# Jaureguy760/HaploHyped-VarAwareML

Measured on AMD Instinct MI355X. Metric: variants/sec encode+compress, 3M-variant x 2.5k-sample VCF, higher is better.
Workload: dtype u8

## Files before the change

### haplohyped_varawareml_amd/csrc/api.hip

```cpp
#include "common.h"
#include <chrono>
#include <vector>
#include <stdarg.h>
#include <stdio.h>
#include <string.h>
#include <stdlib.h>

static thread_local char g_err[512] = "";

void hhgt_set_error(const char *fmt, ...)
{
    va_list ap;
    va_start(ap, fmt);
    vsnprintf(g_err, sizeof(g_err), fmt, ap);
    va_end(ap);
}

extern "C" const char *hhgt_last_error(void) { return g_err; }
extern "C" const char *hhgt_version(void) { return "hhgt 0.1 (gfx950)"; }

extern "C" int hhgt_device_count(void)
{
    int n = 0;
    if (hipGetDeviceCount(&n) != hipSuccess) return 0;
// ... 68 lines not shown
    }
    if (rc == HHGT_OK) rc = c->counters.ensure(sizeof(DevCounters));
    if (rc != HHGT_OK) {
        hhgt_ctx_destroy(c);
        return rc;
    }
    *out = c;
    return HHGT_OK;
}

extern "C" void hhgt_ctx_destroy(hhgt_ctx *c)
{
    if (!c) return;
    hipSetDevice(c->device);
    hipDeviceSynchronize();
    DevBuf *bufs[] = {&c->slots, &c->counts, &c->prefix, &c->nl, &c->scan_tmp, &c->l_soff, &c->l_lend, &c->l_pos,
                      &c->l_refalt, &c->l_flags, &c->l_keep, &c->l_kidx, &c->l_cnew, &c->l_crun, &c->k_soff,
                      &c->k_lend, &c->k_meta, &c->redo_list, &c->redo_flag, &c->run_first, &c->run_names,
                      &c->counters, &c->cursor, &c->result, &c->dec_bad, &c->oh_ovl, &c->oh_lut, &c->crc_x2n,
                      &c->ld_bits};
    for (DevBuf *b : bufs) b->release();
    for (auto &w : c->cw) {
        DevBuf *wb[] = {&w.lz_scratch, &w.lz_csize, &w.lz_flags, &w.fr_bsize, &w.fr_csize, &w.fr_flags};
        for (DevBuf *b : wb) b->release();
        if (w.lz_done) hipEventDestroy(w.lz_done);
        if (w.fr_done) hipEventDestroy(w.fr_done);
    }
    if (c->h_counters) hipHostFree(c->h_counters);
    if (c->h_result_pinned) hipHostFree(c->h_result_pinned);
    for (auto &p : c->pending) {
        hipEventDestroy(p.a);
// ... 217 lines not shown
        return HHGT_ERR_ARG;
    }
    if (L->S > 0 && !d_G) {
        hhgt_set_error("encode: d_G is NULL");
        return HHGT_ERR_ARG;
    }
    const int rc = parse_region_host(region, rf);
    rf->keep_multi = c->keep_multi;
    return rc;
}

static int encode_stage_index(hhgt_ctx *c, const uint8_t *text, uint64_t nbytes, uint32_t n_regions, uint32_t min_line, uint32_t S,
                              DevCounters *cnt, hipStream_t st)
{
    TRY(c->slots.ensure((size_t)n_regions * INDEX_CAP * 4));
    TRY(c->counts.ensure((size_t)n_regions * 4));
    TRY(c->prefix.ensure(((size_t)n_regions + 1) * 4));
    TRY(c->scan_tmp.ensure(2 * scan_tmp_elems(n_regions) * 4));
    TRY(launch_index_newlines(text, nbytes, c->slots.as<uint32_t>(), c->counts.as<uint32_t>(), n_regions, min_line, S, c->index_mode, cnt, st));
    TRY(launch_scan_exclusive_u32_pair(c->counts.as<uint32_t>(), c->prefix.as<uint32_t>(), nullptr, nullptr, n_regions,
                                       c->scan_tmp.as<uint32_t>(), c->scan_tmp.cap / 4, st));
    return HHGT_OK;
}

static int encode_stage_rest(hhgt_ctx *c, const uint8_t *text, uint64_t nbytes, uint32_t n_regions, uint32_t max_lines,
                             const RegionFilter &rf, const LayoutDev &L, const uint64_t *d_cursor, void *d_G, void *d_P, uint32_t *d_start, uint32_t *d_stop,
                             uint8_t *d_ref, uint8_t *d_alt, DevCounters *cnt, hipStream_t st)
{
    const uint32_t *d_nlines = c->prefix.as<uint32_t>() + n_regions;
    const size_t nl4 = ((size_t)max_lines + 1) * 4;
    TRY(c->nl.ensure(nl4));
    TRY(c->scan_tmp.ensure(2 * scan_tmp_elems(max_lines) * 4));
    DevBuf *per_line[] = {&c->l_soff, &c->l_lend, &c->l_pos, &c->l_refalt, &c->l_flags, &c->l_keep,
                          &c->l_kidx, &c->l_cnew, &c->l_crun, &c->k_soff, &c->k_lend, &c->k_meta,
                          &c->redo_list, &c->redo_flag};
    for (DevBuf *b : per_line) TRY(b->ensure(nl4));
    TRY(c->run_first.ensure(MAX_CHROM_RUNS * 8));
    TRY(c->run_names.ensure(MAX_CHROM_RUNS * 32));
    {
        StageTimer t(c, st, HHGT_STAGE_INDEX);
        TRY(launch_compact_newlines(c->slots.as<uint32_t>(), c->counts.as<uint32_t>(), c->prefix.as<uint32_t>(),
                                    n_regions, c->nl.as<uint32_t>(), max_lines, st));
        t.stop();
    }
    if (max_lines == 0) return HHGT_OK;
    {
        StageTimer t(c, st, HHGT_STAGE_FIXED);
        TRY(launch_parse_fixed(text, nbytes, c->nl.as<uint32_t>(), d_nlines, max_lines, rf, L.S,
                               c->l_soff.as<uint32_t>(), c->l_lend.as<uint32_t>(), c->l_pos.as<uint32_t>(),
                               c->l_refalt.as<uint32_t>(), c->l_flags.as<uint32_t>(), c->l_keep.as<uint32_t>(),
                               c->l_cnew.as<uint32_t>(), c->index_mode, cnt, st));
        TRY(launch_scan_exclusive_u32_pair(c->l_keep.as<uint32_t>(), c->l_kidx.as<uint32_t>(), c->l_cnew.as<uint32_t>(),
                                           c->l_crun.as<uint32_t>(), max_lines, c->scan_tmp.as<uint32_t>(), c->scan_tmp.cap / 4, st));
        TRY(launch_compact_kept(text, nbytes, c->nl.as<uint32_t>(), d_nlines, max_lines, c->l_soff.as<uint32_t>(),
                                c->l_lend.as<uint32_t>(), c->l_pos.as<uint32_t>(), c->l_refalt.as<uint32_t>(),
                                c->l_flags.as<uint32_t>(), c->l_kidx.as<uint32_t>(), c->l_crun.as<uint32_t>(),
                                c->k_soff.as<uint32_t>(), c->k_lend.as<uint32_t>(), c->k_meta.as<uint32_t>(),
                                c->redo_list.as<uint32_t>(), c->redo_flag.as<uint32_t>(), c->run_first.as<uint64_t>(), c->run_names.as<uint8_t>(),
                                MAX_CHROM_RUNS, d_cursor, L.v_capacity, L.ring, d_start, d_stop, d_ref, d_alt, cnt, d_P != nullptr, st));
        t.stop();
    }
    if (L.S > 0) {
        StageTimer t(c, st, HHGT_STAGE_ENCODE);
// ... 463 lines not shown
    TRY(planes_columns(lay, col0, n_cols, &L, &pg));
    const uint64_t chunk_nbytes = (uint64_t)L.Sc * L.Vc * 2ull, col_bytes = chunk_nbytes * L.n_sc;
    const uint8_t *g = d_G ? static_cast<const uint8_t *>(d_G) + (uint64_t)col0 * col_bytes : nullptr;
    return compress_impl(c, g, d_P, pg, (uint64_t)n_cols * L.n_sc, chunk_nbytes, 2, 8192, format, d_dst, dst_cap, d_chunk_off, total_bytes,
                         stream);
}

extern "C" int hhgt_reserve(hhgt_ctx *c, uint64_t text_bytes, uint32_t max_lines, uint64_t n_chunks, uint64_t chunk_nbytes, int typesize,
                            int blocksize)
{
    if (!c) return HHGT_ERR_ARG;
    HIP_TRY(hipSetDevice(c->device));
    if (text_bytes) {
        const uint32_t n_regions = (uint32_t)((text_bytes + 1 + INDEX_REGION - 1) / INDEX_REGION);
        TRY(c->slots.ensure((size_t)n_regions * INDEX_CAP * 4));
        TRY(c->counts.ensure((size_t)n_regions * 4));
        TRY(c->prefix.ensure(((size_t)n_regions + 1) * 4));
        const size_t st_el = scan_tmp_elems(n_regions) > scan_tmp_elems(max_lines) ? scan_tmp_elems(n_regions) : scan_tmp_elems(max_lines);
        TRY(c->scan_tmp.ensure(2 * st_el * 4));
        const size_t nl4 = ((size_t)max_lines + 1) * 4;
        TRY(c->nl.ensure(nl4));
        DevBuf *per_line[] = {&c->l_soff, &c->l_lend, &c->l_pos, &c->l_refalt, &c->l_flags, &c->l_keep, &c->l_kidx, &c->l_cnew, &c->l_crun,
                              &c->k_soff, &c->k_lend, &c->k_meta, &c->redo_list, &c->redo_flag};
        for (DevBuf *b : per_line) TRY(b->ensure(nl4));
        TRY(c->run_first.ensure(MAX_CHROM_RUNS * 8));
        TRY(c->run_names.ensure(MAX_CHROM_RUNS * 32));
        TRY(c->result.ensure(sizeof(hhgt_encode_result)));
    }
    if (n_chunks) {
        TRY(check_codec_args(chunk_nbytes, typesize, blocksize, HHGT_BLOSC2));
        blocksize = effective_blocksize(chunk_nbytes, typesize, blocksize);
        uint32_t nblocks, nwaves;
        size_t slot;
        codec_geometry(chunk_nbytes, typesize, blocksize, &nblocks, &nwaves, &slot);
        const uint64_t n_streams = n_chunks * nblocks * nwaves;
        hhgt_ctx::CodecWs &w = c->cw[0];
        TRY(w.lz_scratch.ensure((size_t)n_streams * slot));
// ... 71 lines not shown
        HIP_TRY(hipStreamDestroy(reinterpret_cast<hipStream_t>(stream)));
    }
    return HHGT_OK;
}

extern "C" int hhgt_set_index_mode(hhgt_ctx *c, int mode)
{
    if (!c || mode < -1 || mode > 2) {
        hhgt_set_error("index mode must be -1 (default), 0 (scan), 1 (hop) or 2 (walk)");
        return HHGT_ERR_ARG;
    }
    c->index_mode = mode;
    return HHGT_OK;
}

extern "C" int hhgt_set_keep_multiallelic(hhgt_ctx *c, int on)
{
    if (!c) return HHGT_ERR_ARG;
    c->keep_multi = on ? 1 : 0;
    return HHGT_OK;
}

__global__ void k_count_nonzero_u32(const uint32_t *__restrict__ v, uint64_t n, unsigned long long *out)
{
    uint64_t i = (uint64_t)blockIdx.x * blockDim.x + threadIdx.x;
    const unsigned long long m = __ballot(i < n && v[i] != 0u);
    if ((threadIdx.x & 63u) == 0u && m) atomicAdd(out, (unsigned long long)__builtin_popcountll(m));
}

extern "C" int hhgt_inflate_members(hhgt_ctx *c, const void *d_src, uint64_t src_bytes, const uint64_t *d_comp_off,
// ... 263 lines not shown
```

### haplohyped_varawareml_amd/csrc/common.h

```cpp
#pragma once
#include <hip/hip_runtime.h>
#include <stdint.h>
#include <stddef.h>
#include <string>
#include <vector>
#include "../../include/hhgt.h"

#define HHGT_WAVE 64
#ifdef HHGT_ENC_PRIO
#define HHGT_WAVE_PRIO() __builtin_amdgcn_s_setprio(HHGT_ENC_PRIO)
#else
#define HHGT_WAVE_PRIO()
#endif

#ifdef __HIPCC__
__device__ __forceinline__ uint32_t wave_scan_sum_dpp(uint32_t x, uint32_t lane)
{
    x += (uint32_t)__builtin_amdgcn_update_dpp(0, (int)x, 0x111, 0xf, 0xf, false);
    x += (uint32_t)__builtin_amdgcn_update_dpp(0, (int)x, 0x112, 0xf, 0xf, false);
    x += (uint32_t)__builtin_amdgcn_update_dpp(0, (int)x, 0x114, 0xf, 0xf, false);
    x += (uint32_t)__builtin_amdgcn_update_dpp(0, (int)x, 0x118, 0xf, 0xf, false);
    const uint32_t t0 = (uint32_t)__builtin_amdgcn_readlane((int)x, 15);
    const uint32_t t1 = (uint32_t)__builtin_amdgcn_readlane((int)x, 31) + t0;
    const uint32_t t2 = (uint32_t)__builtin_amdgcn_readlane((int)x, 47) + t1;
// ... 97 lines not shown
    *bi = rem - (rem / g.bpr) * g.bpr;
}

struct DevBuf {
    void *p = nullptr;
    size_t cap = 0;
    int ensure(size_t bytes);
    void release();
    template <typename T> T *as() const { return reinterpret_cast<T *>(p); }
};

struct hhgt_ctx {
    int device = 0;
    hipDeviceProp_t prop;
    DevBuf slots, counts, prefix, nl, scan_tmp;
    DevBuf l_soff, l_lend, l_pos, l_refalt, l_flags, l_keep, l_kidx, l_cnew, l_crun;
    DevBuf k_soff, k_lend, k_meta, redo_list, redo_flag, run_first, run_names;
    DevBuf counters;
    DevBuf cursor;
    DevBuf result;
    struct CodecWs {
        DevBuf lz_scratch, lz_csize, lz_flags, fr_bsize, fr_csize, fr_flags;
        uint32_t lz_tag = 0;
        hipEvent_t lz_done = nullptr, fr_done = nullptr;
        bool fr_pending = false;
    } cw[2];
    uint64_t cmp_seq = 0;
    hipStream_t frame_stream = nullptr;
    DevBuf dec_bad, oh_ovl, oh_lut, crc_x2n;
    DevBuf ld_bits;
// ... 19 lines not shown
    hhgt_ctx *ctx;
    hipStream_t st;
    int stage;
    hipEvent_t a = nullptr, b = nullptr;
    StageTimer(hhgt_ctx *c, hipStream_t s, int stage_);
    void stop();
};
int hhgt_profile_collect(hhgt_ctx *ctx);

int launch_scan_exclusive_u32(const uint32_t *d_in, uint32_t *d_out, uint64_t n, uint32_t *d_tmp,
                              size_t tmp_elems, hipStream_t st);
int launch_scan_exclusive_u32_pair(const uint32_t *in_a, uint32_t *out_a, const uint32_t *in_b, uint32_t *out_b, uint64_t n,
                                   uint32_t *d_tmp, size_t tmp_elems, hipStream_t st);
size_t scan_tmp_elems(uint64_t n);

int launch_index_newlines(const uint8_t *d_text, uint64_t n, uint32_t *d_slots, uint32_t *d_counts,
                          uint32_t n_regions, uint32_t min_line, uint32_t S, int mode, DevCounters *d_cnt, hipStream_t st);
int index_mode_default();
int launch_compact_newlines(const uint32_t *d_slots, const uint32_t *d_counts, const uint32_t *d_prefix,
                            uint32_t n_regions, uint32_t *d_nl, uint32_t max_lines, hipStream_t st);
int launch_parse_fixed(const uint8_t *d_text, uint64_t n, const uint32_t *d_nl, const uint32_t *d_nlines,
                       uint32_t max_lines, const RegionFilter &region, uint32_t S, uint32_t *l_soff, uint32_t *l_lend,
                       uint32_t *l_pos, uint32_t *l_refalt, uint32_t *l_flags, uint32_t *l_keep,
                       uint32_t *l_cnew, int mode, DevCounters *d_cnt, hipStream_t st);
int launch_compact_kept(const uint8_t *d_text, uint64_t n, const uint32_t *d_nl, const uint32_t *d_nlines, uint32_t max_lines,
                        const uint32_t *l_soff, const uint32_t *l_lend,
                        const uint32_t *l_pos, const uint32_t *l_refalt, const uint32_t *l_flags,
                        const uint32_t *l_kidx, const uint32_t *l_crun, uint32_t *k_soff, uint32_t *k_lend,
                        uint32_t *k_meta, uint32_t *redo_list, uint32_t *redo_flag, uint64_t *run_first, uint8_t *run_names,
                        uint32_t max_runs, const uint64_t *d_cursor, uint64_t v_capacity, uint32_t ring, uint32_t *d_start,
                        uint32_t *d_stop, uint8_t *d_ref, uint8_t *d_alt, DevCounters *d_cnt, bool strided, hipStream_t st);

int launch_encode_tiles(const uint8_t *d_text, uint64_t n, const uint32_t *k_soff, const uint32_t *k_meta,
                        uint32_t n_lines_bound, const uint64_t *d_cursor, LayoutDev lay, int8_t *d_G,
                        uint32_t *redo_list, uint32_t *redo_flag, DevCounters *d_cnt, hipStream_t st);
int launch_encode_general(const uint8_t *d_text, uint64_t n, const uint32_t *k_soff, const uint32_t *k_lend,
// ... 57 lines not shown
```

### haplohyped_varawareml_amd/csrc/index.hip

```cpp
#include "common.h"

typedef uint32_t u32x4_unaligned __attribute__((ext_vector_type(4), aligned(1)));
typedef uint32_t u32x4_t __attribute__((ext_vector_type(4)));

__device__ __forceinline__ uint32_t nl_mask4(uint32_t x)
{
    uint32_t t = x ^ 0x0A0A0A0Au;
    uint32_t z = ~(((t & 0x7F7F7F7Fu) + 0x7F7F7F7Fu) | t | 0x7F7F7F7Fu);
    return (((z >> 7) * 0x01020408u) >> 24) & 0xFu;
}

__global__ __launch_bounds__(256) void k_index_newlines(const uint8_t *__restrict__ text, uint64_t n,
                                                        uint32_t *__restrict__ slots,
                                                        uint32_t *__restrict__ counts, uint32_t n_regions,
                                                        DevCounters *cnt)
{
    HHGT_WAVE_PRIO();
    const uint32_t lane = threadIdx.x & 63u;
    const uint32_t r = blockIdx.x * 4u + (threadIdx.x >> 6);
    if (r >= n_regions) return;
    const bool virt = n > 0 && text[n - 1] != '\n';
    const uint64_t rbase = (uint64_t)r * INDEX_REGION;
    uint32_t *my = slots + (size_t)r * INDEX_CAP;
    uint32_t wcount = 0;
// ... 61 lines not shown
    const uint32_t q = (off >> 2) & 3u;
    const uint32_t d = q == 0u ? v.x : (q == 1u ? v.y : (q == 2u ? v.z : v.w));
    return ((uint32_t)__builtin_amdgcn_readlane((int)d, (int)(off >> 4)) >> (8u * (off & 3u))) & 0xFFu;
}

__device__ __forceinline__ uint32_t head_kth(uint32_t m16, uint32_t cum, uint32_t k)
{
    const unsigned long long b = __builtin_amdgcn_ballot_w64(cum < k && cum + (uint32_t)__popc(m16) >= k);
    const int l = __builtin_ctzll(b);
    uint32_t m = (uint32_t)__builtin_amdgcn_readlane((int)m16, l);
    const uint32_t r = k - (uint32_t)__builtin_amdgcn_readlane((int)cum, l);
    for (uint32_t i = 1; i < r; ++i) m &= m - 1u;
    return 16u * (uint32_t)l + (uint32_t)__builtin_ctz(m);
}

#ifndef WALK_BATCH
#define WALK_BATCH 1
#endif
#ifndef WALK_PF
#define WALK_PF 0
#endif
template <int U, bool WALK>
__global__ __launch_bounds__(256) void k_index_hop(const uint8_t *__restrict__ text, uint64_t n, uint32_t *__restrict__ slots,
                                                   uint32_t *__restrict__ counts, uint32_t n_regions, uint32_t skip, uint32_t S,
                                                   DevCounters *cnt, uint32_t HOP_K)
{
    HHGT_WAVE_PRIO();
    const uint32_t lane = threadIdx.x & 63u;
    const uint32_t w = (uint32_t)__builtin_amdgcn_readfirstlane((int)(blockIdx.x * 4u + (threadIdx.x >> 6)));
    const uint32_t r_first = w * HOP_K;
    if (r_first >= n_regions) return;
    const uint32_t r_cnt = n_regions - r_first < HOP_K ? n_regions - r_first : HOP_K;
    const bool virt = n > 0 && text[n - 1] != '\n';
    const uint64_t beg = (uint64_t)r_first * INDEX_REGION;
    uint64_t endw = beg + (uint64_t)r_cnt * INDEX_REGION;
    if (endw > n + 1) endw = n + 1;
    const uint64_t last_term = virt ? n : n - 1;
    uint32_t cntv = 0;
    bool overflow = false;
    uint64_t pos = beg;
    uint64_t cand = 0, fb = 0;
    bool have_cand = false;
    uint64_t est_len = 0, pf_wb = 0;
    bool pf_valid = false;
    u32x4_t pf = u32x4_t{0u, 0u, 0u, 0u};
    auto record = [&](uint64_t q) {
        const uint32_t rr = (uint32_t)(q / INDEX_REGION), local = rr - r_first;
        const uint32_t c = (uint32_t)__builtin_amdgcn_readlane((int)cntv, (int)local);
        if (c < INDEX_CAP) {
            if (lane == 0) slots[(size_t)rr * INDEX_CAP + c] = (uint32_t)q;
        } else
            overflow = true;
        cntv += lane == local ? 1u : 0u;
    };
    bool no_batch = false, bat_off = false;
    uint32_t bat_fail = 0;
    uint64_t head_p = 0;
    bool cand_batch = false;
    bool rehead = false;
    while (have_cand || pos < endw) {
        if (WALK && WALK_BATCH && have_cand && !no_batch && !bat_off && est_len != 0ull && cand >= 40ull && cand + 3ull * est_len + 216ull <= n) {
            const uint32_t g = lane >> 4, li = lane & 15u;
            const uint64_t L0 = est_len;
            const uint8_t *wbase = text + (cand - 40ull);
            const uint64_t voff = (uint64_t)g * L0 + 16ull * li;
// ... 26 lines not shown
#pragma unroll
            for (uint32_t i = 0; i < 8u; ++i) m9 = i < r1 ? (m9 & (m9 - 1u)) : m9;
            const uint32_t j9 = (uint32_t)__builtin_ctz(m9 | 0x10000u) & 15u;
            const uint32_t pw = (uint32_t)__builtin_amdgcn_update_dpp(0, (int)v.w, 0x111, 0xf, 0xf, false);
            const uint32_t ptb = (uint32_t)__builtin_amdgcn_update_dpp(0, (int)tbm, 0x111, 0xf, 0xf, false);
            const uint32_t tb20 = (tbm << 4) | (ptb >> 12);
            const bool tab8 = ((tb20 >> (j9 + 1u)) & 1u) != 0u;
            const uint32_t ix = j9 + 2u, di = ix >> 2;
            const uint32_t w0 = di == 0u ? pw : (di == 1u ? v.x : (di == 2u ? v.y : (di == 3u ? v.z : v.w)));
            const uint32_t w1 = di == 0u ? v.x : (di == 1u ? v.y : (di == 2u ? v.z : v.w));
            const uint32_t gt2 = __builtin_amdgcn_alignbyte(w1, w0, ix & 3u) & 0xFFFFu;
            const bool ok9 = has9 && tab8 && gt2 == 0x5447u;
            const uint32_t t9 = l0 + j9;
            const unsigned long long b9 = __builtin_amdgcn_ballot_w64(ok9);
            uint64_t expected = cand, fbx = fb, exp_head = head_p;
            bool exp_batch = cand_batch;
            bool stop = false, handed = false;
            uint32_t advanced = 0;
#pragma unroll
            for (int k = 0; k < 4; ++k) {
                if (stop || handed) continue;
                const uint64_t nlpos = cand - 40ull + (uint64_t)k * L0 + og[k];
                const bool cr = vg[k] && og[k] != 0u && head_byte(v, 256u * (uint32_t)k + og[k] - 1u) == '\r';
                if (!vg[k] || nlpos != expected || cr) {
                    handed = true;
                    continue;
                }
                exp_head = expected;
                exp_batch = true;
                if (expected >= endw) {
                    stop = true;
                    continue;
                }
                const uint32_t bits = (uint32_t)(b9 >> (16 * k)) & 0xFFFFu;
                if (bits == 0u || ((nl2 >> (16 * k)) & 0xFFFFull) != 0ull) {
                    have_cand = false;
                    pos = expected;
                    handed = true;
                    expected = ~0ull;
                    continue;
                }
                record(expected);
                ++advanced;
                const int l9 = 16 * k + __builtin_ctz(bits);
                const uint32_t t9s = (uint32_t)__builtin_amdgcn_readlane((int)t9, l9);
                const uint64_t soff = cand - 40ull + (uint64_t)k * L0 + t9s + 1ull;
                const uint64_t nxt = soff + 4ull * S - 1ull;
                est_len = nxt - expected;
                expected = nxt;
                fbx = soff + 2ull * S - 17ull;
            }
            if (stop) break;
            if (expected != ~0ull) {
                if (expected > last_term) {
                    have_cand = false;
                    pos = fbx;
                    if (pos > last_term) pos = last_term;
                } else {
                    cand = expected;
                    fb = fbx > last_term ? last_term : fbx;
                    have_cand = true;
                }
                head_p = exp_head;
                cand_batch = exp_batch;
            }
            no_batch = handed;
            bat_fail = advanced ? 0u : bat_fail + 1u;
            bat_off = bat_fail >= 2u;
            continue;
        }
        no_batch = false;
        bool found = false, nb_have = false, have_head = false;
        uint32_t nb_reg = 0, ho = 15u;
        uint64_t p = 0;
        u32x4_t hd = u32x4_t{0u, 0u, 0u, 0u};
        if (WALK && have_cand) {
            have_cand = false;
            uint32_t c15 = 0, c14 = 0;
            const bool use_pf = pf_valid && cand >= pf_wb + 15ull && cand <= pf_wb + 79ull;
            pf_valid = false;
            if (use_pf || cand + 1009ull <= n) {
                if (use_pf) {
                    hd = pf;
                    ho = (uint32_t)(cand - pf_wb);
                } else
                    hd = *reinterpret_cast<const u32x4_unaligned *>(text + (cand - 15ull) + 16ull * lane);
                const uint64_t pred = cand + est_len;
                if (WALK_PF && est_len != 0ull && pred + 977ull <= n && cand < endw) {
// ... 2 lines not shown
                    pf_valid = true;
                }
                c15 = head_byte(hd, ho);
                c14 = head_byte(hd, ho - 1u);
                have_head = true;
            } else if (cand < n) {
                c15 = text[cand];
                c14 = text[cand - 1];
            } else if (cand == n && virt) {
                c15 = 0x0Au;
                c14 = text[n - 1];
            }
            if (c15 == 0x0Au && c14 != '\r') {
                found = true;
                p = cand;
            } else if (cand_batch) {
                cand_batch = false;
                rehead = true;
                found = true;
                have_head = false;
                p = head_p;
            } else {
                pos = fb;
                continue;
            }
        } else {
        const uint64_t a0 = pos & ~15ull;
        uint32_t any[U];
        u32x4_t v[U];
#pragma unroll
// ... 43 lines not shown
                    if (j < 15u && g0 + 16 <= n) {
                        const uint32_t k = j + 1u, dw = k >> 2;
                        const uint32_t xd = dw == 0u ? x0 : (dw == 1u ? x1 : (dw == 2u ? x2 : x3));
                        nb_reg = (xd >> (8u * (k & 3u))) & 0xFFu;
                        nb_have = true;
                    }
                }
            }
        }
        if (!found) {
            pos = a0 + (uint64_t)U * 1024u;
            continue;
        }
        }
        if (!rehead) {
            if (p >= endw) break;
            record(p);
        } else
            no_batch = true;
        rehead = false;
        bool hopped = false;
        if (WALK) {
            if (!have_head && p >= 15ull && p + 1009ull <= n) {
                hd = *reinterpret_cast<const u32x4_unaligned *>(text + (p - 15ull) + 16ull * lane);
                have_head = true;
            }
            if (have_head) {
                const uint64_t wb = p - (uint64_t)ho;
                const uint32_t nb = head_byte(hd, ho + 1u);
                const uint32_t l0 = 16u * lane;
                const uint32_t keep = l0 > ho ? 0xFFFFu : (l0 + 15u <= ho ? 0u : (0xFFFFu << (ho - l0 + 1u)) & 0xFFFFu);
                if (nb == '#' || nb == 0x0Au) {
// ... 6 lines not shown
                        const int l = __builtin_ctzll(nlb);
                        pos = wb + 16ull * (uint64_t)l + (uint64_t)__builtin_ctz((uint32_t)__builtin_amdgcn_readlane((int)nlm, l));
                        hopped = true;
                    } else {
                        const uint32_t tbm = eq_mask16(hd, 0x09090909u) & keep;
                        const uint32_t tc = (uint32_t)__popc(tbm);
                        const uint32_t incl = wave_scan_sum_dpp(tc, lane);
                        const uint32_t total = (uint32_t)__builtin_amdgcn_readlane((int)incl, 63);
                        if (total >= 9u) {
                            const uint32_t t8 = head_kth(tbm, incl - tc, 8u), t9 = head_kth(tbm, incl - tc, 9u);
                            const uint64_t soff = wb + t9 + 1ull;
                            const uint64_t lo = soff + 2ull * S - 17ull;
                            const bool gt = t9 - t8 == 3u && head_byte(hd, t8 + 1u) == 'G' && head_byte(hd, t8 + 2u) == 'T';
                            if (gt && soff + 4ull * S - 1ull <= last_term) {
                                cand = soff + 4ull * S - 1ull;
                                fb = lo;
                                have_cand = true;
                                est_len = cand - p;
                                head_p = p;
                                cand_batch = false;
                            } else {
                                pos = lo;
                            }
                            hopped = true;
                        }
                    }
                }
            }
        }
        if (!hopped) {
            uint32_t nb = 0x0Au;
            if (nb_have) nb = nb_reg;
            else if (p + 1 < n) nb = text[p + 1];
            pos = p + 1 + ((nb == '#' || nb == 0x0Au || nb == '\r') ? 0u : skip);
        }
        if (pos > last_term) pos = p + 1 > last_term ? p + 1 : last_term;
        if (have_cand && fb > last_term) fb = p + 1 > last_term ? p + 1 : last_term;
    }
    if (overflow && lane == 0) atomicAdd(&cnt->err_density, 1ull);
    if (lane < r_cnt) counts[r_first + lane] = cntv < INDEX_CAP ? cntv : INDEX_CAP;
}

__global__ __launch_bounds__(256) void k_compact_newlines(const uint32_t *__restrict__ slots,
                                                          const uint32_t *__restrict__ counts,
                                                          const uint32_t *__restrict__ prefix,
                                                          uint32_t n_regions, uint32_t *__restrict__ nl,
                                                          uint32_t max_lines)
{
    HHGT_WAVE_PRIO();
    uint32_t r = blockIdx.x * blockDim.x + threadIdx.x;
    if (r >= n_regions) return;
    uint32_t c = counts[r], p = prefix[r];
    const uint32_t *my = slots + (size_t)r * INDEX_CAP;
    for (uint32_t k = 0; k < c && p + k < max_lines; ++k) nl[p + k] = my[k];
}

__global__ __launch_bounds__(256) void k_parse_fixed(const uint8_t *__restrict__ text, uint64_t n,
                                                     const uint32_t *__restrict__ nl, const uint32_t *__restrict__ d_nlines,
                                                     uint32_t max_lines, const RegionFilter rfv, uint32_t S,
                                                     uint32_t *__restrict__ l_soff, uint32_t *__restrict__ l_lend,
                                                     uint32_t *__restrict__ l_pos, uint32_t *__restrict__ l_refalt,
                                                     uint32_t *__restrict__ l_flags, uint32_t *__restrict__ l_keep,
                                                     uint32_t *__restrict__ l_cnew, DevCounters *cnt, uint32_t hop_skip)
{
    HHGT_WAVE_PRIO();
    __shared__ uint32_t stage[256][17];
    const RegionFilter *rf = &rfv;
    const uint32_t i = blockIdx.x * blockDim.x + threadIdx.x;
    const uint32_t n_found = *d_nlines;
    const uint32_t n_lines = n_found < max_lines ? n_found : max_lines;
    if (i == 0) {
        cnt->n_lines = n_found;
        cnt->err_lines = n_found > max_lines ? (unsigned long long)(n_found - max_lines) : 0ull;
    }
    if (blockIdx.x * blockDim.x >= n_lines) {
        if (i < max_lines) l_keep[i] = l_cnew[i] = 0u;
        return;
    }
    uint32_t flags = 0;
    uint32_t s = 0, e = 0;
    bool staged = false;
    if (i < n_lines) {
        s = i ? nl[i - 1] + 1u : 0u;
        e = nl[i];
        staged = (uint64_t)s + 64ull <= n;
        if (staged) {
            u32x4_unaligned c[4];
#pragma unroll
            for (int k = 0; k < 4; ++k) c[k] = *reinterpret_cast<const u32x4_unaligned *>(text + s + 16 * k);
#pragma unroll
            for (int k = 0; k < 4; ++k) {
                stage[threadIdx.x][4 * k + 0] = c[k].x;
                stage[threadIdx.x][4 * k + 1] = c[k].y;
                stage[threadIdx.x][4 * k + 2] = c[k].z;
                stage[threadIdx.x][4 * k + 3] = c[k].w;
            }
        }
    }
    __syncthreads();
    const uint8_t *mine = reinterpret_cast<const uint8_t *>(stage[threadIdx.x]);
    auto rd = [&](uint32_t x) -> uint32_t { return (staged && x - s < 64u) ? (uint32_t)mine[x - s] : (uint32_t)text[x]; };
    uint32_t soff = 0, pos0 = 0, refalt = 0, gtidx = 0, stride = 0;
    if (i < n_lines) {
        if (e > s && rd(e - 1u) == '\r') --e;
        soff = e;
        if (e > s && rd(s) != '#') {
            flags = LF_RECORD;
            uint32_t fs[10];
            uint32_t nf = 0;
            uint32_t p = s;
            fs[0] = s;
            while (p < e && nf < 9) {
                if (rd(p) == '\t') fs[++nf] = p + 1;
                ++p;
            }
            bool bad = false;
            uint32_t fe[9];
#pragma unroll
            for (int k = 0; k < 9; ++k) fe[k] = (uint32_t)k < nf ? fs[k + 1] - 1u : e;
            if (nf < 7 || (S > 0 && nf < 9)) bad = true;
            if (!bad) {
                unsigned long long pos = 0;
                if (fe[1] == fs[1]) bad = true;
                for (uint32_t q = fs[1]; q < fe[1]; ++q) {
                    uint32_t c = rd(q);
                    if (c < '0' || c > '9') {
                        bad = true;
                        break;
                    }
// ... 17 lines not shown
                        bool snp = reflen == 1 && altlen == 1 && (a == 'A' || a == 'C' || a == 'G' || a == 'T');
                        if (rf->keep_multi && reflen == 1 && altlen > 1 && (altlen & 1u)) {
                            snp = true;
                            for (uint32_t q = 0; snp && q < altlen; ++q) {
                                const uint32_t ch = rd(fs[4] + q);
                                snp = (q & 1u) ? ch == ',' : (ch == 'A' || ch == 'C' || ch == 'G' || ch == 'T');
                            }
                        }
                        if (!snp)
                            flags |= LF_DROP_FILTER;
                        else {
                            pos0 = (uint32_t)(pos - 1ull);
                            refalt = rd(fs[3]) | (a << 8);
                            if (S > 0) {
                                uint32_t q = fs[8], k = 0;
                                bool found = false;
                                while (q <= fe[8]) {
                                    uint32_t q2 = q;
                                    while (q2 < fe[8] && rd(q2) != ':') ++q2;
                                    if (q2 - q == 2 && rd(q) == 'G' && rd(q + 1u) == 'T') {
                                        found = true;
                                        break;
                                    }
                                    ++k;
                                    q = q2 + 1;
                                }
                                if (!found || k > 0xFFFu) bad = true;
                                gtidx = k;
                                soff = fs[9];
                                if (!bad) {
                                    flags |= LF_KEEP;
                                    if (k == 0 && fe[8] - fs[8] == 2 && e - soff == 4u * S - 1u) flags |= LF_FAST;
// ... 2 lines not shown
                                        if (wd >= 5u && wd <= 8u) stride = wd;
                                    }
                                }
                            } else {
                                flags |= LF_KEEP;
                            }
                        }
                    }
                }
            }
            if (bad) flags = LF_RECORD | LF_MALFORMED;
            bool cnew = true;
            if (i > 0) {
                uint32_t ps = i > 1 ? nl[i - 2] + 1u : 0u;
                uint32_t pe = nl[i - 1];
                const bool pstaged = threadIdx.x > 0u && (uint64_t)ps + 64ull <= n;
                const uint8_t *prev = reinterpret_cast<const uint8_t *>(stage[threadIdx.x > 0u ? threadIdx.x - 1u : 0u]);
                auto rdp = [&](uint32_t x) -> uint32_t { return (pstaged && x - ps < 64u) ? (uint32_t)prev[x - ps] : (uint32_t)text[x]; };
                if (pe > ps && rdp(ps) != '#') {
                    uint32_t q = 0;
                    cnew = false;
                    for (;;) {
                        uint32_t a = fs[0] + q < e ? rd(fs[0] + q) : '\t';
                        uint32_t b = ps + q < pe ? rdp(ps + q) : '\t';
                        if (a != b) {
                            cnew = true;
                            break;
                        }
                        if (a == '\t') break;
                        ++q;
                    }
                }
            }
// ... 131 lines not shown
{
    static const int m = [] {
        if (const char *e = getenv("HHGT_INDEX_MODE")) return atoi(e);
        if (const char *e = getenv("HHGT_INDEX_HOP")) return atoi(e) ? 2 : 0;
        return 2;
    }();
    return m < 0 ? 0 : (m > 2 ? 2 : m);
}

static uint32_t index_hop_skip(uint32_t min_line, int mode)
{
    if (mode < 0) mode = index_mode_default();
    return mode && min_line >= 1536u ? min_line - 16u : 0u;
}

int launch_index_newlines(const uint8_t *d_text, uint64_t n, uint32_t *d_slots, uint32_t *d_counts,
                          uint32_t n_regions, uint32_t min_line, uint32_t S, int mode, DevCounters *d_cnt, hipStream_t st)
{
    if (mode < 0) mode = index_mode_default();
    if (const uint32_t skip = index_hop_skip(min_line, mode)) {
        const bool walk = mode >= 2 && S > 0;
        const uint32_t k_walk = (n_regions + 8191u) / 8192u;
        uint32_t K = walk ? (k_walk < 6u ? 6u : k_walk) : 6u;
        K = K > 64u ? 64u : K;
#define HOP_LAUNCH(U, W)                                                                                                      \
    hipLaunchKernelGGL((k_index_hop<U, W>), dim3(((n_regions + K - 1) / K + 3) / 4), dim3(256), 0, st, d_text, n, d_slots, d_counts, \
                       n_regions, skip, S, d_cnt, K)
        if (min_line >= 4096u) {
            if (walk) HOP_LAUNCH(5, true);
            else HOP_LAUNCH(5, false);
        } else {
            if (walk) HOP_LAUNCH(3, true);
            else HOP_LAUNCH(3, false);
        }
#undef HOP_LAUNCH
        HIP_TRY(hipGetLastError());
        return HHGT_OK;
    }
    hipLaunchKernelGGL(k_index_newlines, dim3((n_regions + 3) / 4), dim3(256), 0, st, d_text, n, d_slots,
                       d_counts, n_regions, d_cnt);
    HIP_TRY(hipGetLastError());
    return HHGT_OK;
}

int launch_compact_newlines(const uint32_t *d_slots, const uint32_t *d_counts, const uint32_t *d_prefix,
                            uint32_t n_regions, uint32_t *d_nl, uint32_t max_lines, hipStream_t st)
{
    hipLaunchKernelGGL(k_compact_newlines, dim3((n_regions + 255) / 256), dim3(256), 0, st, d_slots, d_counts,
                       d_prefix, n_regions, d_nl, max_lines);
    HIP_TRY(hipGetLastError());
    return HHGT_OK;
}

int launch_parse_fixed(const uint8_t *d_text, uint64_t n, const uint32_t *d_nl, const uint32_t *d_nlines,
                       uint32_t max_lines, const RegionFilter &region, uint32_t S, uint32_t *l_soff, uint32_t *l_lend,
                       uint32_t *l_pos, uint32_t *l_refalt, uint32_t *l_flags, uint32_t *l_keep,
                       uint32_t *l_cnew, int mode, DevCounters *d_cnt, hipStream_t st)
{
    if (max_lines == 0) return HHGT_OK;
    if (mode < 0) mode = index_mode_default();
    uint32_t hop_skip = index_hop_skip(S ? 2u * S + 17u : 0u, mode);
    if (hop_skip && mode >= 2) hop_skip = 0xFFFFFFFFu;
    hipLaunchKernelGGL(k_parse_fixed, dim3((max_lines + 255) / 256), dim3(256), 0, st, d_text, n, d_nl, d_nlines,
                       max_lines, region, S, l_soff, l_lend, l_pos, l_refalt, l_flags, l_keep, l_cnew, d_cnt, hop_skip);
    HIP_TRY(hipGetLastError());
    return HHGT_OK;
}

int launch_compact_kept(const uint8_t *d_text, uint64_t n, const uint32_t *d_nl, const uint32_t *d_nlines, uint32_t max_lines,
                        const uint32_t *l_soff, const uint32_t *l_lend,
                        const uint32_t *l_pos, const uint32_t *l_refalt, const uint32_t *l_flags,
                        const uint32_t *l_kidx, const uint32_t *l_crun, uint32_t *k_soff, uint32_t *k_lend,
                        uint32_t *k_meta, uint32_t *redo_list, uint32_t *redo_flag, uint64_t *run_first, uint8_t *run_names,
                        uint32_t max_runs, const uint64_t *d_cursor, uint64_t v_capacity, uint32_t ring, uint32_t *d_start,
                        uint32_t *d_stop, uint8_t *d_ref, uint8_t *d_alt, DevCounters *d_cnt, bool strided, hipStream_t st)
{
    if (max_lines == 0) return HHGT_OK;
    hipLaunchKernelGGL(k_compact_kept, dim3((max_lines + 255) / 256), dim3(256), 0, st, d_text, n, d_nl, d_nlines, max_lines,
// ... 6 lines not shown
```

Before: 152.4 million.

## Pass GT-offset hints from newline walker to fixed-field parser

The walking newline indexer already finds the FORMAT/GT field offset for each line. It now records that offset as a per-line hint, carries it across region boundaries, and compacts it alongside the newline positions. The fixed-field parser uses a valid hint to stage only 32 bytes instead of 64, scan just the first 5 tab-separated fields, and skip the FORMAT GT search. This adds a hints buffer, extra writes in the indexer and compaction kernels, and a cross-region stitching step that must stay consistent with the walker's logic. The carriage-return check was also changed.

```diff
diff --git a/haplohyped_varawareml_amd/csrc/api.hip b/haplohyped_varawareml_amd/csrc/api.hip
--- a/haplohyped_varawareml_amd/csrc/api.hip
+++ b/haplohyped_varawareml_amd/csrc/api.hip
@@ -106,7 +106,7 @@
     if (!c) return;
     hipSetDevice(c->device);
     hipDeviceSynchronize();
-    DevBuf *bufs[] = {&c->slots, &c->counts, &c->prefix, &c->nl, &c->scan_tmp, &c->l_soff, &c->l_lend, &c->l_pos,
+    DevBuf *bufs[] = {&c->slots, &c->hints, &c->l_hint, &c->counts, &c->prefix, &c->nl, &c->scan_tmp, &c->l_soff, &c->l_lend, &c->l_pos,
                       &c->l_refalt, &c->l_flags, &c->l_keep, &c->l_kidx, &c->l_cnew, &c->l_crun, &c->k_soff,
                       &c->k_lend, &c->k_meta, &c->redo_list, &c->redo_flag, &c->run_first, &c->run_names,
                       &c->counters, &c->cursor, &c->result, &c->dec_bad, &c->oh_ovl, &c->oh_lut, &c->crc_x2n,
@@ -354,10 +354,12 @@
                               DevCounters *cnt, hipStream_t st)
 {
     TRY(c->slots.ensure((size_t)n_regions * INDEX_CAP * 4));
+    TRY(c->hints.ensure(index_hints_bytes(n_regions)));
     TRY(c->counts.ensure((size_t)n_regions * 4));
     TRY(c->prefix.ensure(((size_t)n_regions + 1) * 4));
     TRY(c->scan_tmp.ensure(2 * scan_tmp_elems(n_regions) * 4));
-    TRY(launch_index_newlines(text, nbytes, c->slots.as<uint32_t>(), c->counts.as<uint32_t>(), n_regions, min_line, S, c->index_mode, cnt, st));
+    TRY(launch_index_newlines(text, nbytes, c->slots.as<uint32_t>(), c->hints.as<uint32_t>(), c->counts.as<uint32_t>(), n_regions, min_line, S,
+                              c->index_mode, &c->hint_k, cnt, st));
     TRY(launch_scan_exclusive_u32_pair(c->counts.as<uint32_t>(), c->prefix.as<uint32_t>(), nullptr, nullptr, n_regions,
                                        c->scan_tmp.as<uint32_t>(), c->scan_tmp.cap / 4, st));
     return HHGT_OK;
@@ -371,7 +373,7 @@
     const size_t nl4 = ((size_t)max_lines + 1) * 4;
     TRY(c->nl.ensure(nl4));
     TRY(c->scan_tmp.ensure(2 * scan_tmp_elems(max_lines) * 4));
-    DevBuf *per_line[] = {&c->l_soff, &c->l_lend, &c->l_pos, &c->l_refalt, &c->l_flags, &c->l_keep,
+    DevBuf *per_line[] = {&c->l_hint, &c->l_soff, &c->l_lend, &c->l_pos, &c->l_refalt, &c->l_flags, &c->l_keep,
                           &c->l_kidx, &c->l_cnew, &c->l_crun, &c->k_soff, &c->k_lend, &c->k_meta,
                           &c->redo_list, &c->redo_flag};
     for (DevBuf *b : per_line) TRY(b->ensure(nl4));
@@ -379,14 +381,14 @@
     TRY(c->run_names.ensure(MAX_CHROM_RUNS * 32));
     {
         StageTimer t(c, st, HHGT_STAGE_INDEX);
-        TRY(launch_compact_newlines(c->slots.as<uint32_t>(), c->counts.as<uint32_t>(), c->prefix.as<uint32_t>(),
-                                    n_regions, c->nl.as<uint32_t>(), max_lines, st));
+        TRY(launch_compact_newlines(c->slots.as<uint32_t>(), c->hints.as<uint32_t>(), c->counts.as<uint32_t>(), c->prefix.as<uint32_t>(),
+                                    n_regions, c->nl.as<uint32_t>(), c->l_hint.as<uint32_t>(), max_lines, c->hint_k, st));
         t.stop();
     }
     if (max_lines == 0) return HHGT_OK;
     {
         StageTimer t(c, st, HHGT_STAGE_FIXED);
-        TRY(launch_parse_fixed(text, nbytes, c->nl.as<uint32_t>(), d_nlines, max_lines, rf, L.S,
+        TRY(launch_parse_fixed(text, nbytes, c->nl.as<uint32_t>(), c->l_hint.as<uint32_t>(), d_nlines, max_lines, rf, L.S,
                                c->l_soff.as<uint32_t>(), c->l_lend.as<uint32_t>(), c->l_pos.as<uint32_t>(),
                                c->l_refalt.as<uint32_t>(), c->l_flags.as<uint32_t>(), c->l_keep.as<uint32_t>(),
                                c->l_cnew.as<uint32_t>(), c->index_mode, cnt, st));
@@ -880,13 +882,14 @@
     if (text_bytes) {
         const uint32_t n_regions = (uint32_t)((text_bytes + 1 + INDEX_REGION - 1) / INDEX_REGION);
         TRY(c->slots.ensure((size_t)n_regions * INDEX_CAP * 4));
+        TRY(c->hints.ensure(index_hints_bytes(n_regions)));
         TRY(c->counts.ensure((size_t)n_regions * 4));
         TRY(c->prefix.ensure(((size_t)n_regions + 1) * 4));
         const size_t st_el = scan_tmp_elems(n_regions) > scan_tmp_elems(max_lines) ? scan_tmp_elems(n_regions) : scan_tmp_elems(max_lines);
         TRY(c->scan_tmp.ensure(2 * st_el * 4));
         const size_t nl4 = ((size_t)max_lines + 1) * 4;
         TRY(c->nl.ensure(nl4));
-        DevBuf *per_line[] = {&c->l_soff, &c->l_lend, &c->l_pos, &c->l_refalt, &c->l_flags, &c->l_keep, &c->l_kidx, &c->l_cnew, &c->l_crun,
+        DevBuf *per_line[] = {&c->l_hint, &c->l_soff, &c->l_lend, &c->l_pos, &c->l_refalt, &c->l_flags, &c->l_keep, &c->l_kidx, &c->l_cnew, &c->l_crun,
                               &c->k_soff, &c->k_lend, &c->k_meta, &c->redo_list, &c->redo_flag};
         for (DevBuf *b : per_line) TRY(b->ensure(nl4));
         TRY(c->run_first.ensure(MAX_CHROM_RUNS * 8));
@@ -988,6 +991,15 @@
     return HHGT_OK;
 }
 
+extern "C" int hhgt_debug_line_hints(hhgt_ctx *c, uint32_t *out, uint32_t n)
+{
+    if (!c || (n && !out) || (size_t)n * 4 > c->l_hint.cap) return HHGT_ERR_ARG;
+    HIP_TRY(hipSetDevice(c->device));
+    HIP_TRY(hipDeviceSynchronize());
+    if (n) HIP_TRY(hipMemcpy(out, c->l_hint.p, (size_t)n * 4, hipMemcpyDeviceToHost));
+    return HHGT_OK;
+}
+
 extern "C" int hhgt_set_keep_multiallelic(hhgt_ctx *c, int on)
 {
     if (!c) return HHGT_ERR_ARG;
diff --git a/haplohyped_varawareml_amd/csrc/common.h b/haplohyped_varawareml_amd/csrc/common.h
--- a/haplohyped_varawareml_amd/csrc/common.h
+++ b/haplohyped_varawareml_amd/csrc/common.h
@@ -135,6 +135,8 @@
     int device = 0;
     hipDeviceProp_t prop;
     DevBuf slots, counts, prefix, nl, scan_tmp;
+    DevBuf hints, l_hint;
+    uint32_t hint_k = 0;
     DevBuf l_soff, l_lend, l_pos, l_refalt, l_flags, l_keep, l_kidx, l_cnew, l_crun;
     DevBuf k_soff, k_lend, k_meta, redo_list, redo_flag, run_first, run_names;
     DevBuf counters;
@@ -184,12 +186,13 @@
                                    uint32_t *d_tmp, size_t tmp_elems, hipStream_t st);
 size_t scan_tmp_elems(uint64_t n);
 
-int launch_index_newlines(const uint8_t *d_text, uint64_t n, uint32_t *d_slots, uint32_t *d_counts,
-                          uint32_t n_regions, uint32_t min_line, uint32_t S, int mode, DevCounters *d_cnt, hipStream_t st);
+size_t index_hints_bytes(uint32_t n_regions);
+int launch_index_newlines(const uint8_t *d_text, uint64_t n, uint32_t *d_slots, uint32_t *d_hints, uint32_t *d_counts,
+                          uint32_t n_regions, uint32_t min_line, uint32_t S, int mode, uint32_t *hint_k, DevCounters *d_cnt, hipStream_t st);
 int index_mode_default();
-int launch_compact_newlines(const uint32_t *d_slots, const uint32_t *d_counts, const uint32_t *d_prefix,
-                            uint32_t n_regions, uint32_t *d_nl, uint32_t max_lines, hipStream_t st);
-int launch_parse_fixed(const uint8_t *d_text, uint64_t n, const uint32_t *d_nl, const uint32_t *d_nlines,
+int launch_compact_newlines(const uint32_t *d_slots, const uint32_t *d_hints, const uint32_t *d_counts, const uint32_t *d_prefix,
+                            uint32_t n_regions, uint32_t *d_nl, uint32_t *l_hint, uint32_t max_lines, uint32_t hint_k, hipStream_t st);
+int launch_parse_fixed(const uint8_t *d_text, uint64_t n, const uint32_t *d_nl, const uint32_t *l_hint, const uint32_t *d_nlines,
                        uint32_t max_lines, const RegionFilter &region, uint32_t S, uint32_t *l_soff, uint32_t *l_lend,
                        uint32_t *l_pos, uint32_t *l_refalt, uint32_t *l_flags, uint32_t *l_keep,
                        uint32_t *l_cnew, int mode, DevCounters *d_cnt, hipStream_t st);
diff --git a/haplohyped_varawareml_amd/csrc/index.hip b/haplohyped_varawareml_amd/csrc/index.hip
--- a/haplohyped_varawareml_amd/csrc/index.hip
+++ b/haplohyped_varawareml_amd/csrc/index.hip
@@ -99,6 +99,10 @@
     return 16u * (uint32_t)l + (uint32_t)__builtin_ctz(m);
 }
 
+#define HINT_OFF_MASK 0xFFFFu
+#define HINT_VALID 0x10000u
+#define HINT_GT 0x20000u
+
 #ifndef WALK_BATCH
 #define WALK_BATCH 1
 #endif
@@ -107,7 +111,7 @@
 #endif
 template <int U, bool WALK>
 __global__ __launch_bounds__(256) void k_index_hop(const uint8_t *__restrict__ text, uint64_t n, uint32_t *__restrict__ slots,
-                                                   uint32_t *__restrict__ counts, uint32_t n_regions, uint32_t skip, uint32_t S,
+                                                   uint32_t *__restrict__ hints, uint32_t *__restrict__ counts, uint32_t n_regions, uint32_t skip, uint32_t S,
                                                    DevCounters *cnt, uint32_t HOP_K)
 {
     HHGT_WAVE_PRIO();
@@ -126,14 +130,19 @@
     uint64_t pos = beg;
     uint64_t cand = 0, fb = 0;
     bool have_cand = false;
+    uint32_t cand_hint = 0;
+    uint32_t x_pos = ~0u, x_hint = 0;
     uint64_t est_len = 0, pf_wb = 0;
     bool pf_valid = false;
     u32x4_t pf = u32x4_t{0u, 0u, 0u, 0u};
-    auto record = [&](uint64_t q) {
+    auto record = [&](uint64_t q, uint32_t h) {
         const uint32_t rr = (uint32_t)(q / INDEX_REGION), local = rr - r_first;
         const uint32_t c = (uint32_t)__builtin_amdgcn_readlane((int)cntv, (int)local);
         if (c < INDEX_CAP) {
-            if (lane == 0) slots[(size_t)rr * INDEX_CAP + c] = (uint32_t)q;
+            if (lane == 0) {
+                slots[(size_t)rr * INDEX_CAP + c] = (uint32_t)q;
+                if (WALK) hints[(size_t)rr * INDEX_CAP + c] = h;
+            }
         } else
             overflow = true;
         cntv += lane == local ? 1u : 0u;
@@ -190,6 +199,7 @@
             const uint32_t t9 = l0 + j9;
             const unsigned long long b9 = __builtin_amdgcn_ballot_w64(ok9);
             uint64_t expected = cand, fbx = fb, exp_head = head_p;
+            uint32_t exp_hint = cand_hint;
             bool exp_batch = cand_batch;
             bool stop = false, handed = false;
             uint32_t advanced = 0;
@@ -197,7 +207,7 @@
             for (int k = 0; k < 4; ++k) {
                 if (stop || handed) continue;
                 const uint64_t nlpos = cand - 40ull + (uint64_t)k * L0 + og[k];
-                const bool cr = vg[k] && og[k] != 0u && head_byte(v, 256u * (uint32_t)k + og[k] - 1u) == '\r';
+                const bool cr = vg[k] && (og[k] == 0u || head_byte(v, 256u * (uint32_t)k + og[k] - 1u) == '\r');
                 if (!vg[k] || nlpos != expected || cr) {
                     handed = true;
                     continue;
@@ -205,6 +215,8 @@
                 exp_head = expected;
                 exp_batch = true;
                 if (expected >= endw) {
+                    x_pos = (uint32_t)expected;
+                    x_hint = exp_hint;
                     stop = true;
                     continue;
                 }
@@ -216,13 +228,14 @@
                     expected = ~0ull;
                     continue;
                 }
-                record(expected);
+                record(expected, exp_hint);
                 ++advanced;
                 const int l9 = 16 * k + __builtin_ctz(bits);
                 const uint32_t t9s = (uint32_t)__builtin_amdgcn_readlane((int)t9, l9);
                 const uint64_t soff = cand - 40ull + (uint64_t)k * L0 + t9s + 1ull;
                 const uint64_t nxt = soff + 4ull * S - 1ull;
                 est_len = nxt - expected;
+                exp_hint = (uint32_t)(soff - (expected + 1ull)) | HINT_VALID | HINT_GT;
                 expected = nxt;
                 fbx = soff + 2ull * S - 17ull;
             }
@@ -234,6 +247,7 @@
                     if (pos > last_term) pos = last_term;
                 } else {
                     cand = expected;
+                    cand_hint = exp_hint;
                     fb = fbx > last_term ? last_term : fbx;
                     have_cand = true;
                 }
@@ -248,6 +262,7 @@
         no_batch = false;
         bool found = false, nb_have = false, have_head = false;
         uint32_t nb_reg = 0, ho = 15u;
+        uint32_t rec_hint = 0;
         uint64_t p = 0;
         u32x4_t hd = u32x4_t{0u, 0u, 0u, 0u};
         if (WALK && have_cand) {
@@ -280,6 +295,7 @@
             if (c15 == 0x0Au && c14 != '\r') {
                 found = true;
                 p = cand;
+                rec_hint = cand_hint;
             } else if (cand_batch) {
                 cand_batch = false;
                 rehead = true;
@@ -353,8 +369,12 @@
         }
         }
         if (!rehead) {
-            if (p >= endw) break;
-            record(p);
+            if (p >= endw) {
+                x_pos = (uint32_t)p;
+                x_hint = rec_hint;
+                break;
+            }
+            record(p, rec_hint);
         } else
             no_batch = true;
         rehead = false;
@@ -391,6 +411,7 @@
                             const bool gt = t9 - t8 == 3u && head_byte(hd, t8 + 1u) == 'G' && head_byte(hd, t8 + 2u) == 'T';
                             if (gt && soff + 4ull * S - 1ull <= last_term) {
                                 cand = soff + 4ull * S - 1ull;
+                                cand_hint = (uint32_t)(soff - (p + 1ull)) | HINT_VALID | HINT_GT;
                                 fb = lo;
                                 have_cand = true;
                                 est_len = cand - p;
@@ -416,24 +437,52 @@
     }
     if (overflow && lane == 0) atomicAdd(&cnt->err_density, 1ull);
     if (lane < r_cnt) counts[r_first + lane] = cntv < INDEX_CAP ? cntv : INDEX_CAP;
+    if (WALK && lane == 0) {
+        uint32_t *x = hints + (size_t)n_regions * INDEX_CAP + 2u * (size_t)(r_first + r_cnt - 1u);
+        x[0] = x_pos;
+        x[1] = x_hint;
+    }
 }
 
 __global__ __launch_bounds__(256) void k_compact_newlines(const uint32_t *__restrict__ slots,
+                                                          const uint32_t *__restrict__ hints,
                                                           const uint32_t *__restrict__ counts,
                                                           const uint32_t *__restrict__ prefix,
                                                           uint32_t n_regions, uint32_t *__restrict__ nl,
-                                                          uint32_t max_lines)
+                                                          uint32_t *__restrict__ l_hint, uint32_t max_lines, uint32_t hint_k)
 {
     HHGT_WAVE_PRIO();
     uint32_t r = blockIdx.x * blockDim.x + threadIdx.x;
     if (r >= n_regions) return;
     uint32_t c = counts[r], p = prefix[r];
     const uint32_t *my = slots + (size_t)r * INDEX_CAP;
-    for (uint32_t k = 0; k < c && p + k < max_lines; ++k) nl[p + k] = my[k];
+    if (!hint_k) {
+        for (uint32_t k = 0; k < c && p + k < max_lines; ++k) {
+            nl[p + k] = my[k];
+            l_hint[p + k] = 0u;
+        }
+        return;
+    }
+    const uint32_t *myh = hints + (size_t)r * INDEX_CAP;
+    uint32_t first = 0;
+    const uint32_t r0 = r / hint_k * hint_k;
+    if (c != 0u && r0 != 0u) {
+        bool lead = true;
+        for (uint32_t q = r0; lead && q < r; ++q) lead = counts[q] == 0u;
+        if (lead) {
+            const uint32_t *x = hints + (size_t)n_regions * INDEX_CAP + 2u * (size_t)(r0 - 1u);
+            if (x[0] == my[0]) first = x[1];
+        }
+    }
+    for (uint32_t k = 0; k < c && p + k < max_lines; ++k) {
+        nl[p + k] = my[k];
+        l_hint[p + k] = k == 0u ? (myh[0] | first) : myh[k];
+    }
 }
 
 __global__ __launch_bounds__(256) void k_parse_fixed(const uint8_t *__restrict__ text, uint64_t n,
-                                                     const uint32_t *__restrict__ nl, const uint32_t *__restrict__ d_nlines,
+                                                     const uint32_t *__restrict__ nl, const uint32_t *__restrict__ l_hint,
+                                                     const uint32_t *__restrict__ d_nlines,
                                                      uint32_t max_lines, const RegionFilter rfv, uint32_t S,
                                                      uint32_t *__restrict__ l_soff, uint32_t *__restrict__ l_lend,
                                                      uint32_t *__restrict__ l_pos, uint32_t *__restrict__ l_refalt,
@@ -456,30 +505,39 @@
     }
     uint32_t flags = 0;
     uint32_t s = 0, e = 0;
-    bool staged = false;
+    uint32_t staged = 0;
+    uint32_t hoff = 0;
     if (i < n_lines) {
         s = i ? nl[i - 1] + 1u : 0u;
         e = nl[i];
-        staged = (uint64_t)s + 64ull <= n;
+        const uint32_t h = l_hint[i];
+        if ((h & (HINT_VALID | HINT_GT)) == (HINT_VALID | HINT_GT) && S > 0u && e - s == (h & HINT_OFF_MASK) + 4u * S - 1u) hoff = h & HINT_OFF_MASK;
+        const uint32_t want = hoff ? 32u : 64u;
+        staged = (uint64_t)s + want <= n ? want : 0u;
         if (staged) {
-            u32x4_unaligned c[4];
-#pragma unroll
-            for (int k = 0; k < 4; ++k) c[k] = *reinterpret_cast<const u32x4_unaligned *>(text + s + 16 * k);
+            const u32x4_t zero = u32x4_t{0u, 0u, 0u, 0u};
+            u32x4_t c[4];
+#pragma unroll
+            for (int k = 0; k < 4; ++k)
+                c[k] = (k < 2 || staged == 64u) ? u32x4_t(*reinterpret_cast<const u32x4_unaligned *>(text + s + 16 * k)) : zero;
 #pragma unroll
             for (int k = 0; k < 4; ++k) {
-                stage[threadIdx.x][4 * k + 0] = c[k].x;
-                stage[threadIdx.x][4 * k + 1] = c[k].y;
-                stage[threadIdx.x][4 * k + 2] = c[k].z;
-                stage[threadIdx.x][4 * k + 3] = c[k].w;
-            }
-        }
-    }
+                if (k < 2 || staged == 64u) {
+                    stage[threadIdx.x][4 * k + 0] = c[k].x;
+                    stage[threadIdx.x][4 * k + 1] = c[k].y;
+                    stage[threadIdx.x][4 * k + 2] = c[k].z;
+                    stage[threadIdx.x][4 * k + 3] = c[k].w;
+                }
+            }
+        }
+    }
+    stage[threadIdx.x][16] = staged;
     __syncthreads();
     const uint8_t *mine = reinterpret_cast<const uint8_t *>(stage[threadIdx.x]);
-    auto rd = [&](uint32_t x) -> uint32_t { return (staged && x - s < 64u) ? (uint32_t)mine[x - s] : (uint32_t)text[x]; };
+    auto rd = [&](uint32_t x) -> uint32_t { return x - s < staged ? (uint32_t)mine[x - s] : (uint32_t)text[x]; };
     uint32_t soff = 0, pos0 = 0, refalt = 0, gtidx = 0, stride = 0;
     if (i < n_lines) {
-        if (e > s && rd(e - 1u) == '\r') --e;
+        if (!hoff && e > s && rd(e - 1u) == '\r') --e;
         soff = e;
         if (e > s && rd(s) != '#') {
             flags = LF_RECORD;
@@ -487,9 +545,16 @@
             uint32_t nf = 0;
             uint32_t p = s;
             fs[0] = s;
-            while (p < e && nf < 9) {
+            const uint32_t nf_walk = hoff ? 5u : 9u;
+            while (p < e && nf < nf_walk) {
                 if (rd(p) == '\t') fs[++nf] = p + 1;
                 ++p;
+            }
+            if (hoff) {
+                fs[6] = fs[7] = fs[5];
+                fs[9] = s + hoff;
+                fs[8] = fs[9] - 3u;
+                nf = 9;
             }
             bool bad = false;
             uint32_t fe[9];
@@ -537,8 +602,8 @@
                             refalt = rd(fs[3]) | (a << 8);
                             if (S > 0) {
                                 uint32_t q = fs[8], k = 0;
-                                bool found = false;
-                                while (q <= fe[8]) {
+                                bool found = hoff != 0u;
+                                while (!found && q <= fe[8]) {
                                     uint32_t q2 = q;
                                     while (q2 < fe[8] && rd(q2) != ':') ++q2;
                                     if (q2 - q == 2 && rd(q) == 'G' && rd(q + 1u) == 'T') {
@@ -571,9 +636,9 @@
             if (i > 0) {
                 uint32_t ps = i > 1 ? nl[i - 2] + 1u : 0u;
                 uint32_t pe = nl[i - 1];
-                const bool pstaged = threadIdx.x > 0u && (uint64_t)ps + 64ull <= n;
+                const uint32_t pstaged = threadIdx.x > 0u ? stage[threadIdx.x - 1u][16] : 0u;
                 const uint8_t *prev = reinterpret_cast<const uint8_t *>(stage[threadIdx.x > 0u ? threadIdx.x - 1u : 0u]);
-                auto rdp = [&](uint32_t x) -> uint32_t { return (pstaged && x - ps < 64u) ? (uint32_t)prev[x - ps] : (uint32_t)text[x]; };
+                auto rdp = [&](uint32_t x) -> uint32_t { return x - ps < pstaged ? (uint32_t)prev[x - ps] : (uint32_t)text[x]; };
                 if (pe > ps && rdp(ps) != '#') {
                     uint32_t q = 0;
                     cnew = false;
@@ -735,17 +800,21 @@
     return mode && min_line >= 1536u ? min_line - 16u : 0u;
 }
 
-int launch_index_newlines(const uint8_t *d_text, uint64_t n, uint32_t *d_slots, uint32_t *d_counts,
-                          uint32_t n_regions, uint32_t min_line, uint32_t S, int mode, DevCounters *d_cnt, hipStream_t st)
-{
+size_t index_hints_bytes(uint32_t n_regions) { return (size_t)n_regions * (INDEX_CAP + 2u) * 4u; }
+
+int launch_index_newlines(const uint8_t *d_text, uint64_t n, uint32_t *d_slots, uint32_t *d_hints, uint32_t *d_counts,
+                          uint32_t n_regions, uint32_t min_line, uint32_t S, int mode, uint32_t *hint_k, DevCounters *d_cnt, hipStream_t st)
+{
+    *hint_k = 0;
     if (mode < 0) mode = index_mode_default();
     if (const uint32_t skip = index_hop_skip(min_line, mode)) {
         const bool walk = mode >= 2 && S > 0;
         const uint32_t k_walk = (n_regions + 8191u) / 8192u;
         uint32_t K = walk ? (k_walk < 6u ? 6u : k_walk) : 6u;
         K = K > 64u ? 64u : K;
+        if (walk) *hint_k = K;
 #define HOP_LAUNCH(U, W)                                                                                                      \
-    hipLaunchKernelGGL((k_index_hop<U, W>), dim3(((n_regions + K - 1) / K + 3) / 4), dim3(256), 0, st, d_text, n, d_slots, d_counts, \
+    hipLaunchKernelGGL((k_index_hop<U, W>), dim3(((n_regions + K - 1) / K + 3) / 4), dim3(256), 0, st, d_text, n, d_slots, d_hints, d_counts, \
                        n_regions, skip, S, d_cnt, K)
         if (min_line >= 4096u) {
             if (walk) HOP_LAUNCH(5, true);
@@ -764,16 +833,16 @@
     return HHGT_OK;
 }
 
-int launch_compact_newlines(const uint32_t *d_slots, const uint32_t *d_counts, const uint32_t *d_prefix,
-                            uint32_t n_regions, uint32_t *d_nl, uint32_t max_lines, hipStream_t st)
-{
-    hipLaunchKernelGGL(k_compact_newlines, dim3((n_regions + 255) / 256), dim3(256), 0, st, d_slots, d_counts,
-                       d_prefix, n_regions, d_nl, max_lines);
+int launch_compact_newlines(const uint32_t *d_slots, const uint32_t *d_hints, const uint32_t *d_counts, const uint32_t *d_prefix,
+                            uint32_t n_regions, uint32_t *d_nl, uint32_t *l_hint, uint32_t max_lines, uint32_t hint_k, hipStream_t st)
+{
+    hipLaunchKernelGGL(k_compact_newlines, dim3((n_regions + 255) / 256), dim3(256), 0, st, d_slots, d_hints, d_counts,
+                       d_prefix, n_regions, d_nl, l_hint, max_lines, hint_k);
     HIP_TRY(hipGetLastError());
     return HHGT_OK;
 }
 
-int launch_parse_fixed(const uint8_t *d_text, uint64_t n, const uint32_t *d_nl, const uint32_t *d_nlines,
+int launch_parse_fixed(const uint8_t *d_text, uint64_t n, const uint32_t *d_nl, const uint32_t *l_hint, const uint32_t *d_nlines,
                        uint32_t max_lines, const RegionFilter &region, uint32_t S, uint32_t *l_soff, uint32_t *l_lend,
                        uint32_t *l_pos, uint32_t *l_refalt, uint32_t *l_flags, uint32_t *l_keep,
                        uint32_t *l_cnew, int mode, DevCounters *d_cnt, hipStream_t st)
@@ -782,7 +851,7 @@
     if (mode < 0) mode = index_mode_default();
     uint32_t hop_skip = index_hop_skip(S ? 2u * S + 17u : 0u, mode);
     if (hop_skip && mode >= 2) hop_skip = 0xFFFFFFFFu;
-    hipLaunchKernelGGL(k_parse_fixed, dim3((max_lines + 255) / 256), dim3(256), 0, st, d_text, n, d_nl, d_nlines,
+    hipLaunchKernelGGL(k_parse_fixed, dim3((max_lines + 255) / 256), dim3(256), 0, st, d_text, n, d_nl, l_hint, d_nlines,
                        max_lines, region, S, l_soff, l_lend, l_pos, l_refalt, l_flags, l_keep, l_cnew, d_cnt, hop_skip);
     HIP_TRY(hipGetLastError());
     return HHGT_OK;
```

Result: no change. 151.9 million (-0.3%).
